# therealadityashankar/hey-buddy

Hardware: AMD Instinct MI355X
Metric: audio clips/sec featurized+trained, 1.5 s @16 kHz, 1/2/4/8 GPU (higher is better)
Workload: dtype f32

## Files before the change

hey-buddy_amd/csrc/hbk_augment.hip:

```cpp
#include <algorithm>
#include <cmath>
#include <numeric>
#include <type_traits>
#include <vector>

#include "hbk_common.h"

namespace hbk {
namespace {

constexpr int kT = 23040;
constexpr int kM = kT / 2;
constexpr int kThreads = 1024;
constexpr int kN1 = 16000;
constexpr int kM1 = kN1 / 2;

template <bool INV>
__device__ __forceinline__ cf tw_const(double frac) {
  const double a = (INV ? 2.0 : -2.0) * M_PI * frac;
  return cf{static_cast<float>(cos(a)), static_cast<float>(sin(a))};
}

template <bool INV>
__device__ __forceinline__ void dft3(cf& a, cf& b, cf& c) {
// ... 1314 lines not shown
#endif

struct PitchArgs {
  const float* x;
  int64_t x_stride;
  const int32_t* idx;
  int n;
  float* out;
  int64_t out_stride;
  int L, f_in, f_out, l1, orig, nw, width, target;
  double rate;
  float* y;
  float* taps;
  int2* yr;
  int span;
};

__device__ __forceinline__ int ps_i0(const PitchArgs& a, int t, float& alpha) {
  const float ts = static_cast<float>(static_cast<double>(t) * a.rate);
  const float fl = floorf(ts);
  alpha = ts - fl;
  return static_cast<int>(fl);
}

struct PvClip {
  float d[kPvRows][8];
  float xs[256];
  float gh[2][kPvGh][8];
  int cnt0;
  int lo, hi;
// ... 105 lines not shown
        }
      }
    }
    done = 4 * n4;
  }
  for (int p = done + lane; p < L; p += 128) {
    if (xr[p] != 0.f) {
      lo = min(lo, p);
      hi = max(hi, p);
    }
  }
  if (hi >= 0) {
    atomicMin(&C.lo, lo);
    atomicMax(&C.hi, hi);
  }
}

#ifdef HBK_PHASE_TIMING
#define HBK_PVT(i)                                     \
  do {                                                 \
    const unsigned long long t_ = __builtin_amdgcn_s_memtime(); \
    pvt[i] += t_ - pvt_t0;                             \
    pvt_t0 = t_;                                       \
  } while (0)
#else
#define HBK_PVT(i) \
  do {             \
  } while (0)
#endif

#ifndef HBK_PV_UNROLL_TAIL
#define HBK_PV_UNROLL_TAIL 1
#endif
#ifndef HBK_PV_WAVES
#define HBK_PV_WAVES 4
#endif
__global__ void __launch_bounds__(128 * kPvClips) __attribute__((amdgpu_waves_per_eu(HBK_PV_WAVES)))
ps_vocoder_kernel(PitchArgs a) {
#ifdef HBK_PHASE_TIMING
  unsigned long long pvt[5] = {0, 0, 0, 0, 0}, pvt_t0 = __builtin_amdgcn_s_memtime();
#endif
  extern __shared__ __attribute__((aligned(16))) unsigned char pv_smem[];
  PvShared& sh = *reinterpret_cast<PvShared*>(pv_smem);
  const int tid = threadIdx.x, cl = tid >> 7, lane = tid & 127;
  const int e = min(static_cast<int>(blockIdx.x) * kPvClips + cl, a.n - 1);
  const bool live = static_cast<int>(blockIdx.x) * kPvClips + cl < a.n;
  const float* xr = a.x + static_cast<int64_t>(a.idx[e]) * a.x_stride;
  PvClip& C = sh.c[cl];
  for (int q = tid; q < 256; q += blockDim.x) {
    double sn, cs;
    sincospi(2.0 * q / kPsFft, &sn, &cs);
    sh.tw[q] = cf{static_cast<float>(cs), static_cast<float>(sn)};
    sh.tw64[q][0] = cs;
    sh.tw64[q][1] = -sn;
  }
  if (lane == 0) C.cnt0 = 0;
  if (lane == 0) {
    C.lo = INT_MAX;
    C.hi = -1;
  }
  __syncthreads();
  if (a.span) pv_scan_span(C, xr, a.L, lane);
  int nz = 0;
  for (int q = lane; q < kPsFft; q += 128) {
    const float v = ps_xp(xr, a.L, q);
    C.xs[q] = v;
    nz += v != 0.f;
  }
  if (nz) atomicAdd(&C.cnt0, nz);
  for (int q = tid; q < 3 * 128; q += blockDim.x) {
    const int j = 2 * (q / 128) + 1, kk = min(q % 128, kPsBins - 1), q1 = (kk * j) % kPsFft,
              q2 = (kk * (j + 1)) % kPsFft;
    sh.wt[q / 128][q % 128] = float4{static_cast<float>(sh.tw64[q1][0]), static_cast<float>(sh.tw64[q1][1]),
                                     static_cast<float>(sh.tw64[q2][0]), static_cast<float>(sh.tw64[q2][1])};
  }
  int fb = 1;
  pv_load_rows(a, sh, xr, cl, lane, fb);
// ... 81 lines not shown
    commit(nre, nim, ncnt);
    cntn = cnt;
    polar(na, nm);
    slide_to(nre, nim, ncnt, C.d[sf + 1 - fb]);
    commit(nre, nim, ncnt);
    polar(pa, pm);
  }
  int c = 0;
  cf R = {1.f, 0.f};
  cf Q = {0.f, 0.f};
  int qz = 0;
  const int dq = q7;
  const cf e7 = sh.tw[q7];
  const int jmax = (a.l1 + kPsPad - 1) / kPsHop;
  float* y = a.y + static_cast<int64_t>(e) * a.l1;
  auto frames_of = [&](int lo, int hi, int& tb, int& tl) {
    tb = 0;
    tl = jmax;
    float al;
    if (lo > hi) {
      tl = -1;
      return;
    }
    if (lo > 2 * kPsPad && a.rate < 2.0) {
      const int fz = (lo - kPsPad) / kPsHop - 1;
      int tg = min(static_cast<int>((fz - 2) / a.rate), a.f_out - 1) & ~(kPvGroup - 1);
      while (tg > 0 && ps_i0(a, tg - 1, al) + 2 > fz) tg -= kPvGroup;
      tb = max(tg, 0);
    }
    if (hi < a.L - 1 - 2 * kPsPad) {
      const int fn = min((hi + kPsPad) / kPsHop, a.f_in - 1);
      int t = max(min(a.f_out - 1, static_cast<int>((fn + 1) / a.rate) + 1), 0);
      while (t > 0 && ps_i0(a, t, al) > fn) --t;
      while (t + 1 < a.f_out && ps_i0(a, t + 1, al) <= fn) ++t;
      tl = min(jmax, t + 36);
    }
  };
  int t_beg = 0, t_last = jmax;
  {
    int tb = 0, tl = jmax;
    if (a.span) {
      int lo = INT_MAX, hi = -1;
      for (int i = 0; i < kPvClips; ++i) {
        lo = min(lo, sh.c[i].lo);
        hi = max(hi, sh.c[i].hi);
      }
      frames_of(lo, hi, t_beg, t_last);
      frames_of(C.lo, C.hi, tb, tl);
    }
    if (lane == 0 && live)
      a.yr[e] = tl < tb ? int2{0, 0}
                        : int2{max(kPsHop * tb - kPsPad, 0), min(kPsHop * (tl + 1) - kPsPad, a.l1)};
// ... 811 lines not shown
      a.rate * kPvGroup + 3 > kPvRows) {
    set_error("hbk: pitch shift %d/%d resamples %d -> %d (%d taps): the kernel holds <= %d phases of <= %d taps "
              "(torch_pitch_shift's fast shifts at 16 kHz)", num, den, a.orig, a.nw, 2 * a.width + a.orig,
              kPsPhaseMax, kPsTapMax);
    return HBK_ERR_UNSUPPORTED;
  }
  return HBK_OK;
}

static int64_t ps_bytes(const hbk::PitchArgs& a, int64_t n, int64_t* off) {
  using namespace hbk;
  auto up = [](int64_t b) { return (b + 255) & ~int64_t(255); };
  off[0] = off[1] = off[2] = off[3] = 0;
  off[4] = up(n * a.l1 * 4);
  off[5] = off[4] + up(int64_t(kPsPhaseMax) * kPsTapMax * 4);
  return off[5] + up(n * int64_t(sizeof(int2)));
}

int64_t hbk_pitch_shift_workspace_size(int64_t n, int64_t T, int32_t sample_rate, int32_t num, int32_t den) {
  hbk::PitchArgs a{};
  if (n <= 0 || ps_geometry(T, sample_rate, num, den, a) != HBK_OK) return 0;
  int64_t off[6];
  return ps_bytes(a, n, off);
}

int hbk_pitch_shift(const float* x, int64_t x_stride, int64_t n, const int32_t* idx, int64_t T, int32_t sample_rate,
                    int32_t num, int32_t den, float* out, int64_t out_stride, void* workspace,
                    int64_t workspace_bytes, void* stream) {
  using namespace hbk;
  if (n < 0) return arg_error("negative n");
  if (n == 0) return HBK_OK;
  if (n > 65535) return arg_error("n > 65535 per call");
  if (!x || !idx || !out || !workspace) return arg_error("NULL pointer");
  PitchArgs a{};
  const int rc = ps_geometry(T, sample_rate, num, den, a);
  if (rc != HBK_OK) return rc;
  if (x_stride < T || out_stride < T) return arg_error("stride < T");
  int64_t off[6];
  if (workspace_bytes < ps_bytes(a, n, off)) return arg_error("workspace too small (hbk_pitch_shift_workspace_size)");
  unsigned char* w = static_cast<unsigned char*>(workspace);
  a.x = x;
  a.x_stride = x_stride;
  a.idx = idx;
  a.out = out;
  a.out_stride = out_stride;
  a.n = static_cast<int>(n);
  a.y = reinterpret_cast<float*>(w + off[3]);
  a.taps = reinterpret_cast<float*>(w + off[4]);
  a.yr = reinterpret_cast<int2*>(w + off[5]);
  static const bool span_off = [] {
    const char* s = getenv("HBK_PS_SPAN");
    return s && s[0] == '0';
  }();
  a.span = span_off ? 0 : 1;
  hipStream_t st = as_stream(stream);
  hipLaunchKernelGGL(ps_taps_kernel, dim3(unsigned((a.nw * kPsTapMax + 255) / 256)), dim3(256), 0, st, a);
  HBK_LAUNCH_CHECK("ps_taps_kernel");
  static bool lds_set = false;
  if (!lds_set) {
    HBK_HIP(hipFuncSetAttribute(reinterpret_cast<const void*>(ps_vocoder_kernel),
                                hipFuncAttributeMaxDynamicSharedMemorySize, int(sizeof(PvShared))));
    lds_set = true;
  }
  hipLaunchKernelGGL(ps_vocoder_kernel, dim3(unsigned((n + kPvClips - 1) / kPvClips)), dim3(128 * kPvClips),
                     sizeof(PvShared), st, a);
  HBK_LAUNCH_CHECK("ps_vocoder_kernel");
  const int res_frames = (a.L + a.nw - 1) / a.nw;
  static const bool valu_rs = getenv("HBK_PS_RESAMPLE_VALU") != nullptr;
  if (valu_rs || a.nw > 128) {
    hipLaunchKernelGGL(ps_resample_kernel, dim3(unsigned((res_frames + kPsResFrames - 1) / kPsResFrames), unsigned(n)),
                       dim3(128), 0, st, a);
    HBK_LAUNCH_CHECK("ps_resample_kernel");
// ... 20 lines not shown
```

hey-buddy_amd/csrc/hbk_mlp.hip:

```cpp
#include <algorithm>
#include <cmath>
#include <vector>

#include "hbk_common.h"
#include "hbk_mlp_internal.h"

namespace hbk {
namespace {

typedef float f4 __attribute__((ext_vector_type(4)));

constexpr int kStats = 8;
constexpr float kLnEps = 1e-5f;

constexpr int GBM = 64, GBN = 64, GBK = 16;

template <bool TA, bool TB>
__global__ void __launch_bounds__(256) gemm_kernel(const float* __restrict__ A, const float* __restrict__ B,
                                                   float* __restrict__ C, const float* __restrict__ bias,
                                                   int M, int N, int K, int lda, int ldb, int ldc,
                                                   int accumulate, int k_split) {
  __shared__ float As[GBK][GBM + 4];
  __shared__ float Bs[GBK][GBN + 4];
  const int tid = threadIdx.x, lane = tid & 63, wave = tid >> 6;
// ... 664 lines not shown
  if (!mlp_fused_supported(*p)) {
    set_error("hbk: the evaluation pass covers the fused plans");
    return HBK_ERR_UNSUPPORTED;
  }
  if (rows < 0 || row_offset < 0 || rows + row_offset > (int64_t(1) << 31) / 768) return arg_error("rows out of range");
  if (rows == 0) return HBK_OK;
  if (!pool || n_pool <= 0) return arg_error("empty pool");
  if (label != 0 && label != 1) return arg_error("label must be 0 or 1");
  if (dropout_p < 0.f || dropout_p >= 1.f) return arg_error("dropout_p must be in [0, 1)");
  if (ws_bytes < mlp_eval_ws_floats(*p, rows) * int64_t(sizeof(float))) return arg_error("workspace too small");
  return mlp_eval_count(*p, params, pool, pool_is_f16 != 0, n_pool, idx, rows, row_offset, label,
                        activation_threshold, dropout_p, seed, counts, prob, static_cast<float*>(workspace),
                        as_stream(stream));
}

int hbk_mlp_eval_count_multi(const hbk_mlp_plan* p, const float* params, int32_t n_pools,
                             const void* const* pools, int32_t pools_are_f16, const int64_t* n_pool,
                             const int64_t* rows, const int64_t* row_offsets, const int32_t* labels,
                             const uint64_t* seeds, float* const* counts, float activation_threshold,
                             float dropout_p, void* workspace, int64_t ws_bytes, void* stream) {
  using namespace hbk;
  if (!p || !params || !workspace) return arg_error("NULL pointer");
  if (!mlp_fused_supported(*p)) {
    set_error("hbk: the evaluation pass covers the fused plans");
    return HBK_ERR_UNSUPPORTED;
  }
  if (n_pools < 0 || n_pools > kEvalMaxSeg) return arg_error("n_pools must be in [0, 4]");
  if (n_pools == 0) return HBK_OK;
  if (!pools || !n_pool || !rows || !row_offsets || !labels || !seeds || !counts) return arg_error("NULL array");
  if (dropout_p < 0.f || dropout_p >= 1.f) return arg_error("dropout_p must be in [0, 1)");
// ... 28 lines not shown
```

hey-buddy_amd/csrc/hbk_mlp_fused.hip:

```cpp
#include <hip/hip_runtime.h>

#include <algorithm>
#include <initializer_list>
#include <utility>
#include <cmath>
#include <cstdio>

#include "hbk_common.h"
#include "hbk_mlp_internal.h"

namespace hbk {
namespace {

typedef float f4 __attribute__((ext_vector_type(4)));
typedef _Float16 h4 __attribute__((ext_vector_type(4)));

constexpr int kD = 1536, kL = 96, kH = 64, kH2 = 128;
constexpr int kR = 16;
constexpr int kMaxG = 4;
constexpr int kStats = 8;
constexpr float kLnEps = 1e-5f;
constexpr int kLd = 132;
constexpr int kChunkMax = 384;

// ... 2101 lines not shown
  const float* P;
  int64_t b_hg[kMaxG], b_o[kMaxG], w_o[kMaxG], ln_g[kMaxG], ln_b[kMaxG];
  const _Float16* wc;
  int64_t c_o[kMaxG], c_hg[kMaxG];
  float act_thr;
  float* counts;
  int label;
  float* prob;
  int nseg;
  int seg_tile0[kKvMaxSeg + 1];
  const void* seg_pool[kKvMaxSeg];
  int64_t seg_npool[kKvMaxSeg], seg_rows[kKvMaxSeg], seg_r0[kKvMaxSeg];
  uint64_t seg_seed[kKvMaxSeg];
  float* seg_counts[kKvMaxSeg];
  int seg_label[kKvMaxSeg];
};

__global__ void __launch_bounds__(256) kv_prep_kernel(const float* __restrict__ P, int64_t w0, int64_t g_in,
                                                      int64_t b_in, _Float16* __restrict__ wq, float* c0,
                                                      float* c1) {
  __shared__ double red[2][4];
  const int n = blockIdx.x, tid = threadIdx.x;
  const float* W = P + w0 + int64_t(n) * kD;
  double s0 = 0.0, s1 = 0.0;
  for (int k = 2 * tid; k < kD; k += 512) {
    const float wa = W[k], wb = W[k + 1];
    const float ga = wa * P[g_in + k], gb = wb * P[g_in + k + 1];
    uint32_t hi, lo;
    split_pair(16.f * ga, 16.f * gb, hi, lo);
    *reinterpret_cast<uint32_t*>(wq + int64_t(n) * kD + k) = hi;
// ... 24 lines not shown
#define HBK_KV_NT 1
#endif
typedef uint32_t u32x4 __attribute__((ext_vector_type(4)));
__device__ __forceinline__ uint4 load_rows4(const uint4* p) {
#if HBK_KV_NT
  const u32x4 v = __builtin_nontemporal_load(reinterpret_cast<const u32x4*>(p));
  return uint4{v[0], v[1], v[2], v[3]};
#else
  return *p;
#endif
}

constexpr int kKvPiece = 8;
__device__ __forceinline__ int kv_swz(int n) { return (n >> 1) & 7; }
constexpr int kNetWLd = 104, kAld = 100;
template <bool kF16, int NG, int W>
__global__ void __launch_bounds__(64 * W) kv_gemm_kernel(KvArgs a0) {
  KvArgs a = a0;
  int blk = static_cast<int>(blockIdx.x);
  if (a0.nseg > 0) {
    int sg = 0;
#pragma unroll
    for (int q = 1; q < kKvMaxSeg; ++q) sg += (q < a0.nseg && blk >= a0.seg_tile0[q]) ? 1 : 0;
    blk -= a0.seg_tile0[sg];
    a.pool = a0.seg_pool[sg];
    a.n_pool = a0.seg_npool[sg];
    a.idx = nullptr;
    a.rows = a0.seg_rows[sg];
    a.r0 = a0.seg_r0[sg];
    a.seed = a0.seg_seed[sg];
    a.counts = a0.seg_counts[sg];
    a.label = a0.seg_label[sg];
    a.prob = nullptr;
  }
  constexpr int kWBuf = 3;
  constexpr int kRT = (kF16 && W == 8) ? 2 : 1;
  constexpr int kThr = 64 * W;
  constexpr int kGemmBytes = kWBuf * 2 * kH2 * kKvKC * 2;
  constexpr int kWsBytes = 2 * kH2 * kNetWLd * 2;
  constexpr int kActBytes = W * 16 * kRT * kAld * 4;
  constexpr int kLdsBytes = (kGemmBytes > kWsBytes + kActBytes ? kGemmBytes : kWsBytes + kActBytes) + 16;
  static_assert(kLdsBytes <= 160 * 1024, "one workgroup's LDS");
  __shared__ __attribute__((aligned(16))) unsigned char smem[kLdsBytes];
  auto wb = reinterpret_cast<_Float16 (*)[2][kH2][kKvKC]>(smem);
  float (*stS)[16 * kRT][2] = reinterpret_cast<float (*)[16 * kRT][2]>(smem);
  static_assert(sizeof(float) * W * 16 * kRT * 2 <= kWsBytes, "statistics: below the activation tiles");
#ifndef HBK_KV_DEPTH
#define HBK_KV_DEPTH 2
#endif
  constexpr int kDepth = kF16 ? HBK_KV_DEPTH : 2;
  constexpr int kBGroup = kDepth > 2 ? 2 : 4;
  constexpr int kU = kF16 ? 1 : 2;
  constexpr int kALoads = kRT * 2 * kU;
  constexpr int kTile = W * 16 * kRT;
  constexpr int kDma = 32 / W;
  static_assert(kALoads * (kDepth - 1) + kDma < 16, "the counted waits use vmcnt's low field");
  const int tid = threadIdx.x, lane = tid & 63, wave = tid >> 6, m = lane & 15, kq = lane >> 4;
  const int64_t tile0 = int64_t(blk) * kTile;
  const char* rp[kRT];
  uint32_t rid[kRT];
#pragma unroll
  for (int rt = 0; rt < kRT; ++rt) {
    const int64_t r = min(tile0 + 16 * kRT * wave + 16 * rt + m, a.rows - 1);
    int64_t pr = a.idx ? static_cast<int64_t>(a.idx[r]) : (a.r0 + r) % a.n_pool;
    pr = min(max(pr, int64_t(0)), a.n_pool - 1);
    rp[rt] = static_cast<const char*>(a.pool) + pr * kD * (kF16 ? 2 : 4);
    rid[rt] = static_cast<uint32_t>(a.r0 + r);
  }
  const uint64_t seed = a.seed;
  const uint32_t s0 = static_cast<uint32_t>(seed), s1 = static_cast<uint32_t>(seed >> 32) * 0x27D4EB2Fu;
  const uint32_t thr = static_cast<uint32_t>(a.drop_p * 65536.f + 0.5f);
  const float keep = a.drop_p > 0.f ? 1.f / (1.f - a.drop_p) : 1.f;
  uint4 ar[kDepth][kRT][2][kU];
  auto load_rows = [&](int c, int slot) {
#pragma unroll
    for (int rt = 0; rt < kRT; ++rt)
#pragma unroll
      for (int kb = 0; kb < 2; ++kb) {
        const int k = kKvKC * c + 32 * kb + 8 * kq;
#pragma unroll
        for (int u = 0; u < kU; ++u)
          ar[slot][rt][kb][u] = load_rows4(reinterpret_cast<const uint4*>(rp[rt] + int64_t(k) * (kF16 ? 2 : 4) + 16 * u));
      }
  };
  auto dma_w = [&](int c, int buf) {
#pragma unroll
    for (int j = 0; j < kDma; ++j) {
      const int row8 = kDma * wave + j;
      const int pl = row8 >> 4, n = 8 * (row8 & 15) + (lane >> 3), pc = (lane & 7) ^ kv_swz(n);
      const _Float16* src = a.wq + int64_t(pl) * kH2 * kD + int64_t(n) * kD + kKvKC * c + kKvPiece * pc;
      __builtin_amdgcn_global_load_lds(src, &wb[buf][pl][8 * (row8 & 15)][0], 16, 0, 0);
// ... 20 lines not shown
  for (int cb = 0; cb < kKvChunks; cb += kDepth)
#pragma unroll
  for (int slot = 0; slot < kDepth; ++slot) {
    const int c = cb + slot;
    const int bnext = buf == 0 ? kWBuf - 1 : buf - 1;
    h8 ah[kRT][2], al[kRT][2];
    float t1[kRT], t2[kRT];
#pragma unroll
    for (int rt = 0; rt < kRT; ++rt) t1[rt] = t2[rt] = 0.f;
#pragma unroll
    for (int kb = 0; kb < 2; ++kb)
#pragma unroll
      for (int rt = 0; rt < kRT; ++rt) {
        float v[8];
        if (kF16) {
          const h8 hv = __builtin_bit_cast(h8, ar[slot][rt][kb][0]);
#pragma unroll
          for (int e = 0; e < 8; ++e) v[e] = static_cast<float>(hv[e]);
        } else {
#pragma unroll
          for (int e = 0; e < 8; ++e) v[e] = __builtin_bit_cast(float, (&ar[slot][rt][kb][e >> 2].x)[e & 3]);
        }
        if (!(HBK_KV_ABLATE & 2) && a.drop_p > 0.f) {
          const uint32_t base = rid[rt] * (kD / 2) + ((kKvKC * c + 32 * kb + 8 * kq) >> 1);
#pragma unroll
          for (int e = 0; e < 8; e += 2) {
            const uint32_t hsh = drop_hash(s0, s1, base + (e >> 1));
            v[e] = (hsh & 0xFFFFu) < thr ? 0.f : v[e];
            v[e + 1] = (hsh >> 16) < thr ? 0.f : v[e + 1];
          }
        }
#pragma unroll
        for (int e = 0; e < 8; ++e) {
          t1[rt] += v[e];
          t2[rt] += v[e] * v[e];
        }
// ... 225 lines not shown
  {
    const int r = lane >> 2, c0 = 16 * (lane & 3);
    float wo[16];
#pragma unroll
    for (int q = 0; q < 16; ++q) wo[q] = P[a.w_o[NG - 1] + c0 + q];
    const float bz = P[a.b_o[NG - 1]];
    int ge = 0, gt = 0;
#pragma unroll
    for (int rt = 0; rt < kRT; ++rt) {
      float z = 0.f;
#pragma unroll
      for (int q = 0; q < 16; ++q) z = fmaf(A[(16 * rt + r) * kAld + c0 + q], wo[q], z);
      z += dpp_f<0xB1>(z);
      z += dpp_f<0x4E>(z);
      z += bz;
      const int64_t row = tile0 + 16 * kRT * wave + 16 * rt + r;
      const bool live = row < a.rows && (lane & 3) == 0;
      const float p = sigm_fast(z);
      if (live && a.prob) a.prob[row] = p;
      ge += __popcll(__ballot(live && p >= a.act_thr));
      gt += __popcll(__ballot(live && p > a.act_thr));
    }
    if (lane == 0) {
      if (ge) atomicAdd(&cntS[0], static_cast<float>(ge));
      if (gt) atomicAdd(&cntS[1], static_cast<float>(gt));
    }
  }
  lds_barrier();
  if (tid < 2 && cntS[tid] != 0.f) atomicAdd(a.counts + 2 * a.label + tid, cntS[tid]);
}


// ... 632 lines not shown

int mlp_eval_prepare(const hbk_mlp_plan& p, const float* params, float* ws, hipStream_t s) {
  const int NG = static_cast<int>(p.g.size());
  const EvalWs w = eval_layout(NG);
  const WSplit wsp = make_wsplit(p);
  const int64_t n4 = wsplit_halves(NG) / 16;
  hipLaunchKernelGGL(k0_wsplit_kernel, dim3(unsigned(std::min<int64_t>((n4 + 255) / 256, 256))), dim3(256), 0, s,
                     wsp, params, reinterpret_cast<_Float16*>(ws + w.wsplit), n4);
  HBK_LAUNCH_CHECK("k0_wsplit_kernel");
  hipLaunchKernelGGL(kv_prep_kernel, dim3(kH2), dim3(256), 0, s, params, p.g[0].w_hg, p.ln_in.g, p.ln_in.b,
                     reinterpret_cast<_Float16*>(ws + w.wq), ws + w.c0, ws + w.c1);
  HBK_LAUNCH_CHECK("kv_prep_kernel");
  return HBK_OK;
}

static int mlp_eval_launch(const hbk_mlp_plan& p, const float* params, bool f16, const EvalSeg* seg, int nseg,
                           const int32_t* idx, float act_thr, float drop_p, float* prob, float* ws, hipStream_t s) {
  const int NG = static_cast<int>(p.g.size());
  const EvalWs w = eval_layout(NG);
  const WSplit wsp = make_wsplit(p);
  K2Args kc{};
  set_k2_cache(wsp, NG, reinterpret_cast<const _Float16*>(ws + w.wsplit), kc);
  KvArgs ka{};
  ka.pool = seg[0].pool;
  ka.n_pool = seg[0].n_pool;
  ka.idx = idx;
  ka.rows = seg[0].rows;
  ka.r0 = seg[0].r0;
  ka.wq = reinterpret_cast<const _Float16*>(ws + w.wq);
  ka.c0 = ws + w.c0;
// ... 25 lines not shown
    ka.nseg = nseg;
    tiles = 0;
    for (int i = 0; i < nseg; ++i) {
      ka.seg_tile0[i] = static_cast<int>(tiles);
      ka.seg_pool[i] = seg[i].pool;
      ka.seg_npool[i] = seg[i].n_pool;
      ka.seg_rows[i] = seg[i].rows;
      ka.seg_r0[i] = seg[i].r0;
      ka.seg_seed[i] = seg[i].seed;
      ka.seg_counts[i] = seg[i].counts;
      ka.seg_label[i] = seg[i].label;
      tiles += (seg[i].rows + tile - 1) / tile;
    }
    ka.seg_tile0[nseg] = static_cast<int>(tiles);
  }
  const dim3 grid(static_cast<unsigned>(tiles));
  auto launch = [&](auto kern) { hipLaunchKernelGGL(kern, grid, dim3(64 * waves), 0, s, ka); };
  if (waves == 16) {
    if (NG == 2) launch(kv_gemm_kernel<true, 2, 16>);
    else if (NG == 3) launch(kv_gemm_kernel<true, 3, 16>);
    else launch(kv_gemm_kernel<true, 4, 16>);
  } else if (f16) {
    if (NG == 2) launch(kv_gemm_kernel<true, 2, 8>);
    else if (NG == 3) launch(kv_gemm_kernel<true, 3, 8>);
    else launch(kv_gemm_kernel<true, 4, 8>);
  } else {
    if (NG == 2) launch(kv_gemm_kernel<false, 2, 8>);
    else if (NG == 3) launch(kv_gemm_kernel<false, 3, 8>);
    else launch(kv_gemm_kernel<false, 4, 8>);
  }
// ... 70 lines not shown
```

hey-buddy_amd/csrc/hbk_mlp_internal.h:

```cpp
#pragma once

#include <hip/hip_runtime.h>
#include <stdint.h>

#include <vector>

namespace hbk {

struct Gmlp {
  int in, hid, out;
  int64_t w_hg, b_hg, w_o, b_o;
};
struct Ln {
  int d;
  int64_t g, b;
};

}

struct hbk_mlp_plan {
  int d_in = 0, layer = 0, hid = 0, n_layers = 0;
  hbk::Ln ln_in;
  std::vector<hbk::Gmlp> g;
  std::vector<hbk::Ln> ln;
// ... 20 lines not shown
int64_t mlp_fused_ws_floats(const hbk_mlp_plan& p, int64_t B);
int mlp_fused_step_variant(int64_t B, hipStream_t s);
int mlp_fused_run(const hbk_mlp_plan& p, const float* params, const float* pool32, int64_t n32,
                  const void* pool16, int64_t n16, const int32_t* idx, int64_t idx_stride, int64_t idx_steps,
                  const float* y, int64_t y_stride, int B, const float* state, int parity, const float* sched,
                  int sched_len, float neg_weight, float thr, float act_thr, float drop_p, uint64_t seed,
                  float* bucket, float* prob, float* logit, float* ws, bool train, int flags, hipStream_t s);
int mlp_fused_update(const hbk_mlp_plan& p, float* params, float* bucket, float* m, float* v, float* state,
                     int parity, const float* sched, int sched_len, float lr, float b1, float b2, float eps,
                     float* hist, int hist_cap, float* ws, hipStream_t s);
int64_t mlp_eval_ws_floats(const hbk_mlp_plan& p, int64_t rows);
int mlp_eval_prepare(const hbk_mlp_plan& p, const float* params, float* ws, hipStream_t s);
int mlp_eval_count(const hbk_mlp_plan& p, const float* params, const void* pool, bool f16, int64_t n_pool,
                   const int32_t* idx, int64_t rows, int64_t r0, int label, float act_thr, float drop_p,
                   uint64_t seed, float* counts, float* prob, float* ws, hipStream_t s);
struct EvalSeg {
  const void* pool;
  int64_t n_pool, rows, r0;
  uint64_t seed;
  float* counts;
  int label;
};
constexpr int kEvalMaxSeg = 4;
int mlp_eval_count_multi(const hbk_mlp_plan& p, const float* params, bool f16, const EvalSeg* seg, int nseg,
                         float act_thr, float drop_p, float* ws, hipStream_t s);
int mlp_eval_finish(const float* cv, const float* ct, const double* sizes, float target, float ratio, float* sched,
                    int64_t sched_len, int64_t next_step, float* out, hipStream_t s);
}
```

hey-buddy_amd/heybuddy/_native.py:

```python
from __future__ import annotations

import ctypes
import os
import threading
from typing import Optional

import torch

__all__ = ["HBKError", "HBKUnavailable", "lib", "check", "stream_ptr", "require_device",
           "LIB_PATH"]

LIB_PATH = os.environ.get(
    "HBK_LIB",
    os.path.join(os.path.dirname(os.path.dirname(os.path.abspath(__file__))), "lib", "libhbk.so"),
)


class HBKError(RuntimeError):
    """A libhbk.so entry point returned a non-zero status."""


class HBKUnavailable(HBKError):
    """libhbk.so (or a HIP device) is not available: the HIP path cannot run."""

# ... 74 lines not shown
    "hbk_mlp_fused_supported": (_c_int, [_vp, ctypes.POINTER(ctypes.c_int32)]),
    "hbk_mlp_step_variant": (_c_int, [_vp, _c_int64, _vp, ctypes.POINTER(ctypes.c_int32)]),
    "hbk_mlp_step_fwd_bwd": (_c_int, [_vp, _vp, _vp, _c_int64, _vp, _c_int64, _vp, _c_int64, _vp, _c_int64,
                                      _c_int64, _vp, ctypes.c_int32, _vp, _c_int64, _c_float, _c_float,
                                      _c_float, _c_float, ctypes.c_uint64, _vp, _vp, _c_int64, ctypes.c_int32,
                                      _vp, _c_int64, _vp]),
    "hbk_mlp_step_update": (_c_int, [_vp, _vp, _vp, _vp, _vp, _vp, ctypes.c_int32, _vp, _c_int64, _c_float,
                                     _c_float, _c_float, _c_float, _vp, ctypes.c_int32, _vp, _c_int64, _vp]),
    "hbk_mlp_eval_workspace_size": (_c_int, [_vp, _c_int64, ctypes.POINTER(_c_int64)]),
    "hbk_mlp_eval_prepare": (_c_int, [_vp, _vp, _vp, _c_int64, _vp]),
    "hbk_mlp_eval_count_multi": (_c_int, [_vp, _vp, ctypes.c_int32, _vp, ctypes.c_int32, _vp, _vp, _vp, _vp, _vp,
                                          _vp, _c_float, _c_float, _vp, _c_int64, _vp]),
    "hbk_mlp_eval_count": (_c_int, [_vp, _vp, _vp, ctypes.c_int32, _c_int64, _vp, _c_int64, _c_int64,
                                    ctypes.c_int32, _c_float, _c_float, ctypes.c_uint64, _vp, _vp, _vp, _c_int64,
                                    _vp]),
    "hbk_mlp_eval_finish": (_c_int, [_vp, _vp, ctypes.POINTER(ctypes.c_double), _c_float, _c_float, _vp,
                                     _c_int64, _c_int64, _vp, _vp]),
}


class GraphOp(ctypes.Structure):
    _fields_ = [
        ("kind", ctypes.c_int32), ("kh", ctypes.c_int32), ("kw", ctypes.c_int32),
        ("cin", ctypes.c_int32), ("cout", ctypes.c_int32), ("act", ctypes.c_int32),
        ("alpha", ctypes.c_float), ("weight", _vp), ("bias", _vp),
    ]


def exported_symbols() -> list[str]:
    return list(_PROTOS)
# ... 52 lines not shown
```

hey-buddy_amd/heybuddy/kernels.py:

```python
from __future__ import annotations

import ctypes
import os
import itertools
import threading
from typing import Dict

import numpy as np
import torch

from heybuddy import _native
from heybuddy._native import check, lib, ptr, stream_ptr

__all__ = ["MelPlan", "mel_frames"]

_plans: Dict[int, object] = {}
_plan_ids = itertools.count(1)
_plans_lock = threading.Lock()


def _register(plan) -> int:
    with _plans_lock:
        pid = next(_plan_ids)
        _plans[pid] = plan
# ... 458 lines not shown
        flat = pool.reshape(pool.shape[0], -1)
        if flat.shape[1] != self.d_in or pool.dtype not in (torch.float32, torch.float16) or pool.device != dev \
                or not pool.is_contiguous():
            raise ValueError(f"pool must be a contiguous [n, {self.d_in}] f32 / f16 tensor on {dev}")
        if idx is not None and (idx.dtype != torch.int32 or idx.device != dev or not idx.is_contiguous()
                                or idx.numel() < rows):
            raise ValueError("idx must be a contiguous int32 device tensor of >= rows entries")
        if counts.dtype != torch.float32 or counts.numel() < 4 or counts.device != dev:
            raise ValueError("counts must be a float32 [4] device tensor")
        if prob is not None and (prob.dtype != torch.float32 or prob.numel() < rows or prob.device != dev):
            raise ValueError("prob must be a float32 device tensor of >= rows entries")
        torch.ops.hbk.mlp_eval_count_(params, pool, idx, int(rows), int(row_offset), int(label),
                                      float(activation_threshold), float(dropout_p), _u64_to_i64(seed), counts, prob,
                                      ws, self.id)

    def eval_count_multi(self, params: torch.Tensor, parts, counts: torch.Tensor, ws: torch.Tensor,
                         activation_threshold: float = 0.5, dropout_p: float = 0.0) -> None:
        dev = params.device
        if not 0 < len(parts) <= 4:
            raise ValueError("1 to 4 pools per launch")
        dt = parts[0][0].dtype
        for pool, rows, _, label, which, _ in parts:
            if pool.dtype != dt or pool.dtype not in (torch.float32, torch.float16) or pool.device != dev \
                    or not pool.is_contiguous() or pool.reshape(pool.shape[0], -1).shape[1] != self.d_in:
                raise ValueError(f"pools must be contiguous [n, {self.d_in}] tensors of one dtype on {dev}")
            if label not in (0, 1) or which not in (0, 1) or rows < 0:
                raise ValueError("label / which must be 0 or 1, rows >= 0")
        if counts.dtype != torch.float32 or counts.shape != (2, 4) or counts.device != dev \
                or not counts.is_contiguous():
            raise ValueError("counts must be a contiguous float32 [2, 4] device tensor")
# ... 570 lines not shown
```

include/hbk.h:

```cpp
#ifndef HBK_H
#define HBK_H

#include <stdint.h>

#ifdef __cplusplus
extern "C" {
#endif

typedef enum {
  HBK_OK = 0,
  HBK_ERR_ARG = -1,
  HBK_ERR_HIP = -2,
  HBK_ERR_UNSUPPORTED = -3
} hbk_status;

const char* hbk_version(void);
const char* hbk_last_error(void);
int hbk_device_count(int* count);
int hbk_stream_create_cu_mask(const uint32_t* cu_mask, int n_words, void** stream);
int hbk_stream_destroy(void* stream);

int hbk_profile_mark(int32_t tag, void* stream);

typedef struct hbk_mel_plan hbk_mel_plan;
// ... 95 lines not shown
                         void* workspace, int64_t workspace_bytes, void* stream);
int hbk_mlp_step_update(const hbk_mlp_plan* plan, float* params, float* bucket, float* m, float* v,
                        float* state, int32_t parity, const float* sched, int64_t sched_len, float lr,
                        float beta1, float beta2, float eps, float* history, int32_t history_cap,
                        void* workspace, int64_t workspace_bytes, void* stream);

int hbk_mlp_set_step_scalars(hbk_mlp_plan* plan, const double* dev_scalars);

int hbk_mlp_eval_workspace_size(const hbk_mlp_plan* plan, int64_t rows, int64_t* bytes);
int hbk_mlp_eval_prepare(const hbk_mlp_plan* plan, const float* params, void* workspace, int64_t workspace_bytes,
                         void* stream);
int hbk_mlp_eval_count(const hbk_mlp_plan* plan, const float* params, const void* pool, int32_t pool_is_f16,
                       int64_t n_pool, const int32_t* idx, int64_t rows, int64_t row_offset, int32_t label,
                       float activation_threshold, float dropout_p, uint64_t seed, float* counts, float* prob,
                       void* workspace, int64_t workspace_bytes, void* stream);
int hbk_mlp_eval_count_multi(const hbk_mlp_plan* plan, const float* params, int32_t n_pools,
                             const void* const* pools, int32_t pools_are_f16, const int64_t* n_pool,
                             const int64_t* rows, const int64_t* row_offsets, const int32_t* labels,
                             const uint64_t* seeds, float* const* counts, float activation_threshold,
                             float dropout_p, void* workspace, int64_t workspace_bytes, void* stream);
int hbk_mlp_eval_finish(const float* counts_val, const float* counts_test, const double* sizes,
                        float target_false_positives_per_hour, float adjust_ratio, float* sched, int64_t sched_len,
                        int64_t next_step, float* out, void* stream);

typedef struct hbk_reverb_plan hbk_reverb_plan;

int hbk_reverb_plan_create(int64_t T, hbk_reverb_plan** plan);
int hbk_reverb_plan_destroy(hbk_reverb_plan* plan);

#define HBK_REVERB_SPECTRUM_SLOTS 11536
// ... 57 lines not shown
```

Before: 1.046 million.

## Sort pitch-shift clips by nonzero span and add lap-form MLP eval kernel

Result: faster. 1.070 million (median of 6 runs) (+2.3%).

```diff
diff --git a/hey-buddy_amd/csrc/hbk_augment.hip b/hey-buddy_amd/csrc/hbk_augment.hip
--- a/hey-buddy_amd/csrc/hbk_augment.hip
+++ b/hey-buddy_amd/csrc/hbk_augment.hip
@@ -1352,6 +1352,10 @@
   float* taps;
   int2* yr;
   int span;
+  int2* sp;
+  uint64_t* key;
+  int32_t* ord;
+  int32_t* gord;
 };
 
 __device__ __forceinline__ int ps_i0(const PitchArgs& a, int t, float& alpha) {
@@ -1487,6 +1491,124 @@
     atomicMin(&C.lo, lo);
     atomicMax(&C.hi, hi);
   }
+}
+
+__device__ __forceinline__ void pv_frames_of(const PitchArgs& a, int lo, int hi, int& tb, int& tl) {
+  const int jmax = (a.l1 + kPsPad - 1) / kPsHop;
+  tb = 0;
+  tl = jmax;
+  float al;
+  if (lo > hi) {
+    tl = -1;
+    return;
+  }
+  if (lo > 2 * kPsPad && a.rate < 2.0) {
+    const int fz = (lo - kPsPad) / kPsHop - 1;
+    int tg = min(static_cast<int>((fz - 2) / a.rate), a.f_out - 1) & ~(kPvGroup - 1);
+    while (tg > 0 && ps_i0(a, tg - 1, al) + 2 > fz) tg -= kPvGroup;
+    tb = max(tg, 0);
+  }
+  if (hi < a.L - 1 - 2 * kPsPad) {
+    const int fn = min((hi + kPsPad) / kPsHop, a.f_in - 1);
+    int t = max(min(a.f_out - 1, static_cast<int>((fn + 1) / a.rate) + 1), 0);
+    while (t > 0 && ps_i0(a, t, al) > fn) --t;
+    while (t + 1 < a.f_out && ps_i0(a, t + 1, al) <= fn) ++t;
+    tl = min(jmax, t + 36);
+  }
+}
+
+constexpr int kPsQuant = 360;
+
+__global__ void __launch_bounds__(256) ps_span_kernel(PitchArgs a) {
+  const int lane = threadIdx.x & 63, e = blockIdx.x * 4 + (threadIdx.x >> 6);
+  if (e >= a.n) return;
+  const float* xr = a.x + static_cast<int64_t>(a.idx[e]) * a.x_stride;
+  constexpr int kChunk = 64 * 8;
+  int lo = INT_MAX, hi = -1;
+  for (int p0 = 0; p0 < a.L; p0 += kChunk) {
+    float v[8];
+#pragma unroll
+    for (int j = 0; j < 8; ++j) {
+      const int p = p0 + 64 * j + lane;
+      v[j] = p < a.L ? xr[p] : 0.f;
+    }
+#pragma unroll
+    for (int j = 0; j < 8; ++j)
+      if (v[j] != 0.f) {
+        lo = min(lo, p0 + 64 * j + lane);
+        hi = max(hi, p0 + 64 * j + lane);
+      }
+    if (__any(hi >= 0)) break;
+  }
+  for (int o = 32; o >= 1; o >>= 1) {
+    lo = min(lo, __shfl_xor(lo, o, 64));
+    hi = max(hi, __shfl_xor(hi, o, 64));
+  }
+  if (hi >= 0) {
+    for (int p1 = a.L; p1 > hi + 1; p1 -= kChunk) {
+      float v[8];
+      int h = -1;
+#pragma unroll
+      for (int j = 0; j < 8; ++j) {
+        const int p = p1 - kChunk + 64 * j + lane;
+        v[j] = (p > hi && p < a.L) ? xr[max(p, 0)] : 0.f;
+      }
+#pragma unroll
+      for (int j = 0; j < 8; ++j)
+        if (v[j] != 0.f) h = max(h, p1 - kChunk + 64 * j + lane);
+      if (__any(h >= 0)) {
+        for (int o = 32; o >= 1; o >>= 1) h = max(h, __shfl_xor(h, o, 64));
+        hi = h;
+        break;
+      }
+    }
+  }
+  if (lane == 0) {
+    a.sp[e] = int2{lo, hi};
+    const uint64_t q = hi < 0 ? 0 : 1 + static_cast<uint64_t>(hi / kPsQuant), f = hi < 0 ? 0 : static_cast<uint64_t>(lo);
+    a.key[e] = (q << 40) | (f << 16) | static_cast<uint64_t>(e);
+  }
+}
+
+__global__ void __launch_bounds__(1024) ps_rank_kernel(const uint64_t* __restrict__ key, int n,
+                                                       int32_t* __restrict__ ord) {
+  __shared__ int part[16][64];
+  const int lane = threadIdx.x & 63, w = threadIdx.x >> 6, i = blockIdx.x * 64 + lane;
+  const uint64_t mine = key[min(i, n - 1)];
+  const int per = (n + 15) / 16, j0 = min(w * per, n), j1 = min(j0 + per, n);
+  int below = 0;
+  for (int jb = j0; jb < j1; jb += 64) {
+    const uint64_t kl = jb + lane < j1 ? key[jb + lane] : ~uint64_t(0);
+#pragma unroll
+    for (int q = 0; q < 64; ++q) {
+      const uint32_t hi = __builtin_amdgcn_readlane(static_cast<int>(kl >> 32), q);
+      const uint32_t lo = __builtin_amdgcn_readlane(static_cast<int>(kl), q);
+      below += ((static_cast<uint64_t>(hi) << 32) | lo) < mine;
+    }
+  }
+  part[w][lane] = below;
+  __syncthreads();
+  if (w == 0 && i < n) {
+    int r = 0;
+#pragma unroll
+    for (int q = 0; q < 16; ++q) r += part[q][lane];
+    ord[r] = i;
+  }
+}
+
+__global__ void __launch_bounds__(256) ps_group_kernel(PitchArgs a, int groups) {
+  const int g = blockIdx.x * 256 + threadIdx.x;
+  if (g >= groups) return;
+  int lo = INT_MAX, hi = -1;
+  for (int c = 0; c < kPvClips; ++c) {
+    const int2 s = a.sp[a.ord[min(kPvClips * g + c, a.n - 1)]];
+    lo = min(lo, s.x);
+    hi = max(hi, s.y);
+  }
+  int tb, tl;
+  pv_frames_of(a, lo, hi, tb, tl);
+  const int steps = tl < tb ? 0 : (tl - tb) / kPvGroup + 1;
+  a.key[g] = (static_cast<uint64_t>((1 << 24) - steps) << 16) | static_cast<uint64_t>(g);
 }
 
 #ifdef HBK_PHASE_TIMING
@@ -1516,8 +1638,9 @@
   extern __shared__ __attribute__((aligned(16))) unsigned char pv_smem[];
   PvShared& sh = *reinterpret_cast<PvShared*>(pv_smem);
   const int tid = threadIdx.x, cl = tid >> 7, lane = tid & 127;
-  const int e = min(static_cast<int>(blockIdx.x) * kPvClips + cl, a.n - 1);
-  const bool live = static_cast<int>(blockIdx.x) * kPvClips + cl < a.n;
+  const int slot = (a.sp ? a.gord[blockIdx.x] : static_cast<int>(blockIdx.x)) * kPvClips + cl;
+  const int e = a.sp ? a.ord[min(slot, a.n - 1)] : min(slot, a.n - 1);
+  const bool live = slot < a.n;
   const float* xr = a.x + static_cast<int64_t>(a.idx[e]) * a.x_stride;
   PvClip& C = sh.c[cl];
   for (int q = tid; q < 256; q += blockDim.x) {
@@ -1529,11 +1652,12 @@
   }
   if (lane == 0) C.cnt0 = 0;
   if (lane == 0) {
-    C.lo = INT_MAX;
-    C.hi = -1;
+    const int2 s = a.sp ? a.sp[e] : int2{INT_MAX, -1};
+    C.lo = s.x;
+    C.hi = s.y;
   }
   __syncthreads();
-  if (a.span) pv_scan_span(C, xr, a.L, lane);
+  if (a.span && !a.sp) pv_scan_span(C, xr, a.L, lane);
   int nz = 0;
   for (int q = lane; q < kPsFft; q += 128) {
     const float v = ps_xp(xr, a.L, q);
@@ -1645,28 +1769,7 @@
   const cf e7 = sh.tw[q7];
   const int jmax = (a.l1 + kPsPad - 1) / kPsHop;
   float* y = a.y + static_cast<int64_t>(e) * a.l1;
-  auto frames_of = [&](int lo, int hi, int& tb, int& tl) {
-    tb = 0;
-    tl = jmax;
-    float al;
-    if (lo > hi) {
-      tl = -1;
-      return;
-    }
-    if (lo > 2 * kPsPad && a.rate < 2.0) {
-      const int fz = (lo - kPsPad) / kPsHop - 1;
-      int tg = min(static_cast<int>((fz - 2) / a.rate), a.f_out - 1) & ~(kPvGroup - 1);
-      while (tg > 0 && ps_i0(a, tg - 1, al) + 2 > fz) tg -= kPvGroup;
-      tb = max(tg, 0);
-    }
-    if (hi < a.L - 1 - 2 * kPsPad) {
-      const int fn = min((hi + kPsPad) / kPsHop, a.f_in - 1);
-      int t = max(min(a.f_out - 1, static_cast<int>((fn + 1) / a.rate) + 1), 0);
-      while (t > 0 && ps_i0(a, t, al) > fn) --t;
-      while (t + 1 < a.f_out && ps_i0(a, t + 1, al) <= fn) ++t;
-      tl = min(jmax, t + 36);
-    }
-  };
+  auto frames_of = [&](int lo, int hi, int& tb, int& tl) { pv_frames_of(a, lo, hi, tb, tl); };
   int t_beg = 0, t_last = jmax;
   {
     int tb = 0, tl = jmax;
@@ -2508,13 +2611,17 @@
   off[0] = off[1] = off[2] = off[3] = 0;
   off[4] = up(n * a.l1 * 4);
   off[5] = off[4] + up(int64_t(kPsPhaseMax) * kPsTapMax * 4);
-  return off[5] + up(n * int64_t(sizeof(int2)));
+  off[6] = off[5] + up(n * int64_t(sizeof(int2)));
+  off[7] = off[6] + up(n * int64_t(sizeof(int2)));
+  off[8] = off[7] + up(n * int64_t(sizeof(uint64_t)));
+  off[9] = off[8] + up(n * int64_t(sizeof(int32_t)));
+  return off[9] + up(n * int64_t(sizeof(int32_t)));
 }
 
 int64_t hbk_pitch_shift_workspace_size(int64_t n, int64_t T, int32_t sample_rate, int32_t num, int32_t den) {
   hbk::PitchArgs a{};
   if (n <= 0 || ps_geometry(T, sample_rate, num, den, a) != HBK_OK) return 0;
-  int64_t off[6];
+  int64_t off[10];
   return ps_bytes(a, n, off);
 }
 
@@ -2530,7 +2637,7 @@
   const int rc = ps_geometry(T, sample_rate, num, den, a);
   if (rc != HBK_OK) return rc;
   if (x_stride < T || out_stride < T) return arg_error("stride < T");
-  int64_t off[6];
+  int64_t off[10];
   if (workspace_bytes < ps_bytes(a, n, off)) return arg_error("workspace too small (hbk_pitch_shift_workspace_size)");
   unsigned char* w = static_cast<unsigned char*>(workspace);
   a.x = x;
@@ -2547,9 +2654,26 @@
     return s && s[0] == '0';
   }();
   a.span = span_off ? 0 : 1;
+  const char* pair_env = getenv("HBK_PS_PAIR");
+  const bool pair = a.span && !(pair_env && pair_env[0] == '0');
   hipStream_t st = as_stream(stream);
   hipLaunchKernelGGL(ps_taps_kernel, dim3(unsigned((a.nw * kPsTapMax + 255) / 256)), dim3(256), 0, st, a);
   HBK_LAUNCH_CHECK("ps_taps_kernel");
+  const int groups = static_cast<int>((n + kPvClips - 1) / kPvClips);
+  if (pair) {
+    a.sp = reinterpret_cast<int2*>(w + off[6]);
+    a.key = reinterpret_cast<uint64_t*>(w + off[7]);
+    a.ord = reinterpret_cast<int32_t*>(w + off[8]);
+    a.gord = reinterpret_cast<int32_t*>(w + off[9]);
+    hipLaunchKernelGGL(ps_span_kernel, dim3(unsigned((n + 3) / 4)), dim3(256), 0, st, a);
+    HBK_LAUNCH_CHECK("ps_span_kernel");
+    hipLaunchKernelGGL(ps_rank_kernel, dim3(unsigned((n + 63) / 64)), dim3(1024), 0, st, static_cast<const uint64_t*>(a.key), a.n, a.ord);
+    HBK_LAUNCH_CHECK("ps_rank_kernel");
+    hipLaunchKernelGGL(ps_group_kernel, dim3(unsigned((groups + 255) / 256)), dim3(256), 0, st, a, groups);
+    HBK_LAUNCH_CHECK("ps_group_kernel");
+    hipLaunchKernelGGL(ps_rank_kernel, dim3(unsigned((groups + 63) / 64)), dim3(1024), 0, st, static_cast<const uint64_t*>(a.key), groups, a.gord);
+    HBK_LAUNCH_CHECK("ps_rank_kernel");
+  }
   static bool lds_set = false;
   if (!lds_set) {
     HBK_HIP(hipFuncSetAttribute(reinterpret_cast<const void*>(ps_vocoder_kernel),
diff --git a/hey-buddy_amd/csrc/hbk_mlp.hip b/hey-buddy_amd/csrc/hbk_mlp.hip
--- a/hey-buddy_amd/csrc/hbk_mlp.hip
+++ b/hey-buddy_amd/csrc/hbk_mlp.hip
@@ -702,6 +702,14 @@
                         as_stream(stream));
 }
 
+int hbk_mlp_eval_laps(int64_t rows, int64_t n_pool, int32_t pool_is_f16, int32_t has_idx, int64_t* parts) {
+  using namespace hbk;
+  if (!parts) return arg_error("NULL pointer");
+  if (rows < 0 || n_pool <= 0) return arg_error("rows / n_pool out of range");
+  mlp_eval_lap_plan(rows, n_pool, pool_is_f16 != 0, has_idx != 0, parts);
+  return HBK_OK;
+}
+
 int hbk_mlp_eval_count_multi(const hbk_mlp_plan* p, const float* params, int32_t n_pools,
                              const void* const* pools, int32_t pools_are_f16, const int64_t* n_pool,
                              const int64_t* rows, const int64_t* row_offsets, const int32_t* labels,
diff --git a/hey-buddy_amd/csrc/hbk_mlp_fused.hip b/hey-buddy_amd/csrc/hbk_mlp_fused.hip
--- a/hey-buddy_amd/csrc/hbk_mlp_fused.hip
+++ b/hey-buddy_amd/csrc/hbk_mlp_fused.hip
@@ -2139,6 +2139,7 @@
   uint64_t seg_seed[kKvMaxSeg];
   float* seg_counts[kKvMaxSeg];
   int seg_label[kKvMaxSeg];
+  int lap_tiles;
 };
 
 __global__ void __launch_bounds__(256) kv_prep_kernel(const float* __restrict__ P, int64_t w0, int64_t g_in,
@@ -2193,8 +2194,9 @@
 constexpr int kKvPiece = 8;
 __device__ __forceinline__ int kv_swz(int n) { return (n >> 1) & 7; }
 constexpr int kNetWLd = 104, kAld = 100;
-template <bool kF16, int NG, int W>
+template <bool kF16, int NG, int W, int kLap = 0>
 __global__ void __launch_bounds__(64 * W) kv_gemm_kernel(KvArgs a0) {
+  static_assert(kLap == 0 || (kF16 && W == 8 && kLap == 2), "the lap form: f16 rows, 8 waves of two laps");
   KvArgs a = a0;
   int blk = static_cast<int>(blockIdx.x);
   if (a0.nseg > 0) {
@@ -2213,7 +2215,8 @@
     a.prob = nullptr;
   }
   constexpr int kWBuf = 3;
-  constexpr int kRT = (kF16 && W == 8) ? 2 : 1;
+  constexpr int kRT = kLap ? kLap : (kF16 && W == 8) ? 2 : 1;
+  constexpr int kAT = kLap ? 1 : kRT;
   constexpr int kThr = 64 * W;
   constexpr int kGemmBytes = kWBuf * 2 * kH2 * kKvKC * 2;
   constexpr int kWsBytes = 2 * kH2 * kNetWLd * 2;
@@ -2230,14 +2233,34 @@
   constexpr int kDepth = kF16 ? HBK_KV_DEPTH : 2;
   constexpr int kBGroup = kDepth > 2 ? 2 : 4;
   constexpr int kU = kF16 ? 1 : 2;
-  constexpr int kALoads = kRT * 2 * kU;
+  constexpr int kALoads = kAT * 2 * kU;
   constexpr int kTile = W * 16 * kRT;
   constexpr int kDma = 32 / W;
   static_assert(kALoads * (kDepth - 1) + kDma < 16, "the counted waits use vmcnt's low field");
   const int tid = threadIdx.x, lane = tid & 63, wave = tid >> 6, m = lane & 15, kq = lane >> 4;
   const int64_t tile0 = int64_t(blk) * kTile;
-  const char* rp[kRT];
+  const int64_t lap_s = kLap ? int64_t(blk / max(a.lap_tiles, 1)) * kLap * a.n_pool : 0;
+  const int64_t lap_b = kLap ? int64_t(blk % max(a.lap_tiles, 1)) * (16 * W) + 16 * wave : 0;
+  auto row_of = [&](int rt, int j, bool& live) -> int64_t {
+    if constexpr (kLap > 0) {
+      const int64_t r = lap_s + rt * a.n_pool + lap_b + j;
+      live = lap_b + j < a.n_pool && r < a.rows;
+      return r;
+    } else {
+      const int64_t r = tile0 + 16 * kRT * wave + 16 * rt + j;
+      live = r < a.rows;
+      return r;
+    }
+  };
+  const char* rp[kAT];
   uint32_t rid[kRT];
+  if constexpr (kLap > 0) {
+    const int64_t b = min(lap_b + m, a.n_pool - 1);
+    const int64_t pr = min(max((a.r0 + b) % a.n_pool, int64_t(0)), a.n_pool - 1);
+    rp[0] = static_cast<const char*>(a.pool) + pr * kD * 2;
+#pragma unroll
+    for (int rt = 0; rt < kRT; ++rt) rid[rt] = static_cast<uint32_t>(a.r0 + lap_s + rt * a.n_pool + b);
+  } else {
 #pragma unroll
   for (int rt = 0; rt < kRT; ++rt) {
     const int64_t r = min(tile0 + 16 * kRT * wave + 16 * rt + m, a.rows - 1);
@@ -2246,14 +2269,15 @@
     rp[rt] = static_cast<const char*>(a.pool) + pr * kD * (kF16 ? 2 : 4);
     rid[rt] = static_cast<uint32_t>(a.r0 + r);
   }
+  }
   const uint64_t seed = a.seed;
   const uint32_t s0 = static_cast<uint32_t>(seed), s1 = static_cast<uint32_t>(seed >> 32) * 0x27D4EB2Fu;
   const uint32_t thr = static_cast<uint32_t>(a.drop_p * 65536.f + 0.5f);
   const float keep = a.drop_p > 0.f ? 1.f / (1.f - a.drop_p) : 1.f;
-  uint4 ar[kDepth][kRT][2][kU];
+  uint4 ar[kDepth][kAT][2][kU];
   auto load_rows = [&](int c, int slot) {
 #pragma unroll
-    for (int rt = 0; rt < kRT; ++rt)
+    for (int rt = 0; rt < kAT; ++rt)
 #pragma unroll
       for (int kb = 0; kb < 2; ++kb) {
         const int k = kKvKC * c + 32 * kb + 8 * kq;
@@ -2304,12 +2328,12 @@
       for (int rt = 0; rt < kRT; ++rt) {
         float v[8];
         if (kF16) {
-          const h8 hv = __builtin_bit_cast(h8, ar[slot][rt][kb][0]);
+          const h8 hv = __builtin_bit_cast(h8, ar[slot][kLap ? 0 : rt][kb][0]);
 #pragma unroll
           for (int e = 0; e < 8; ++e) v[e] = static_cast<float>(hv[e]);
         } else {
 #pragma unroll
-          for (int e = 0; e < 8; ++e) v[e] = __builtin_bit_cast(float, (&ar[slot][rt][kb][e >> 2].x)[e & 3]);
+          for (int e = 0; e < 8; ++e) v[e] = __builtin_bit_cast(float, (&ar[slot][kLap ? 0 : rt][kb][e >> 2].x)[e & 3]);
         }
         if (!(HBK_KV_ABLATE & 2) && a.drop_p > 0.f) {
           const uint32_t base = rid[rt] * (kD / 2) + ((kKvKC * c + 32 * kb + 8 * kq) >> 1);
@@ -2565,8 +2589,9 @@
       z += dpp_f<0xB1>(z);
       z += dpp_f<0x4E>(z);
       z += bz;
-      const int64_t row = tile0 + 16 * kRT * wave + 16 * rt + r;
-      const bool live = row < a.rows && (lane & 3) == 0;
+      bool live;
+      const int64_t row = row_of(rt, r, live);
+      live = live && (lane & 3) == 0;
       const float p = sigm_fast(z);
       if (live && a.prob) a.prob[row] = p;
       ge += __popcll(__ballot(live && p >= a.act_thr));
@@ -3229,6 +3254,15 @@
   return HBK_OK;
 }
 
+void mlp_eval_lap_plan(int64_t rows, int64_t n_pool, bool f16, bool has_idx, int64_t part[2]) {
+  part[0] = 0;
+  part[1] = rows;
+  const char* e = getenv("HBK_EVAL_LAPS");
+  if ((e && e[0] == '0') || !f16 || has_idx || n_pool <= 0 || rows <= 0) return;
+  part[0] = rows / (2 * n_pool) * (2 * n_pool);
+  part[1] = rows - part[0];
+}
+
 static int mlp_eval_launch(const hbk_mlp_plan& p, const float* params, bool f16, const EvalSeg* seg, int nseg,
                            const int32_t* idx, float act_thr, float drop_p, float* prob, float* ws, hipStream_t s) {
   const int NG = static_cast<int>(p.g.size());
@@ -3284,6 +3318,26 @@
     }
     ka.seg_tile0[nseg] = static_cast<int>(tiles);
   }
+  if (nseg == 1) {
+    int64_t part[2];
+    mlp_eval_lap_plan(seg[0].rows, seg[0].n_pool, f16, idx != nullptr, part);
+    if (part[0] > 0) {
+      ka.lap_tiles = static_cast<int>((seg[0].n_pool + 127) / 128);
+      ka.rows = part[0];
+      const dim3 lgrid(static_cast<unsigned>(part[0] / (2 * seg[0].n_pool) * ka.lap_tiles));
+      auto llaunch = [&](auto kern) { hipLaunchKernelGGL(kern, lgrid, dim3(512), 0, s, ka); };
+      if (NG == 2) llaunch(kv_gemm_kernel<true, 2, 8, 2>);
+      else if (NG == 3) llaunch(kv_gemm_kernel<true, 3, 8, 2>);
+      else llaunch(kv_gemm_kernel<true, 4, 8, 2>);
+      HBK_LAUNCH_CHECK("kv_gemm_kernel (laps)");
+      ka.r0 += part[0];
+      if (ka.prob) ka.prob += part[0];
+      ka.lap_tiles = 0;
+      ka.rows = part[1];
+      if (part[1] == 0) return HBK_OK;
+      tiles = (part[1] + tile - 1) / tile;
+    }
+  }
   const dim3 grid(static_cast<unsigned>(tiles));
   auto launch = [&](auto kern) { hipLaunchKernelGGL(kern, grid, dim3(64 * waves), 0, s, ka); };
   if (waves == 16) {
diff --git a/hey-buddy_amd/csrc/hbk_mlp_internal.h b/hey-buddy_amd/csrc/hbk_mlp_internal.h
--- a/hey-buddy_amd/csrc/hbk_mlp_internal.h
+++ b/hey-buddy_amd/csrc/hbk_mlp_internal.h
@@ -58,6 +58,7 @@
 int mlp_eval_count(const hbk_mlp_plan& p, const float* params, const void* pool, bool f16, int64_t n_pool,
                    const int32_t* idx, int64_t rows, int64_t r0, int label, float act_thr, float drop_p,
                    uint64_t seed, float* counts, float* prob, float* ws, hipStream_t s);
+void mlp_eval_lap_plan(int64_t rows, int64_t n_pool, bool f16, bool has_idx, int64_t part[2]);
 struct EvalSeg {
   const void* pool;
   int64_t n_pool, rows, r0;
diff --git a/hey-buddy_amd/heybuddy/_native.py b/hey-buddy_amd/heybuddy/_native.py
--- a/hey-buddy_amd/heybuddy/_native.py
+++ b/hey-buddy_amd/heybuddy/_native.py
@@ -112,6 +112,8 @@
     "hbk_mlp_eval_count": (_c_int, [_vp, _vp, _vp, ctypes.c_int32, _c_int64, _vp, _c_int64, _c_int64,
                                     ctypes.c_int32, _c_float, _c_float, ctypes.c_uint64, _vp, _vp, _vp, _c_int64,
                                     _vp]),
+    "hbk_mlp_eval_laps": (_c_int, [_c_int64, _c_int64, ctypes.c_int32, ctypes.c_int32,
+                                   ctypes.POINTER(_c_int64)]),
     "hbk_mlp_eval_finish": (_c_int, [_vp, _vp, ctypes.POINTER(ctypes.c_double), _c_float, _c_float, _vp,
                                      _c_int64, _c_int64, _vp, _vp]),
 }
diff --git a/hey-buddy_amd/heybuddy/kernels.py b/hey-buddy_amd/heybuddy/kernels.py
--- a/hey-buddy_amd/heybuddy/kernels.py
+++ b/hey-buddy_amd/heybuddy/kernels.py
@@ -496,6 +496,13 @@
                                       float(activation_threshold), float(dropout_p), _u64_to_i64(seed), counts, prob,
                                       ws, self.id)
 
+    @staticmethod
+    def eval_laps(rows: int, n_pool: int, f16: bool = True, has_idx: bool = False) -> tuple:
+        parts = (ctypes.c_int64 * 2)()
+        check(lib().hbk_mlp_eval_laps(int(rows), int(n_pool), int(bool(f16)), int(bool(has_idx)), parts),
+              "hbk_mlp_eval_laps")
+        return tuple(int(v) for v in parts)
+
     def eval_count_multi(self, params: torch.Tensor, parts, counts: torch.Tensor, ws: torch.Tensor,
                          activation_threshold: float = 0.5, dropout_p: float = 0.0) -> None:
         dev = params.device
diff --git a/include/hbk.h b/include/hbk.h
--- a/include/hbk.h
+++ b/include/hbk.h
@@ -133,6 +133,7 @@
                        int64_t n_pool, const int32_t* idx, int64_t rows, int64_t row_offset, int32_t label,
                        float activation_threshold, float dropout_p, uint64_t seed, float* counts, float* prob,
                        void* workspace, int64_t workspace_bytes, void* stream);
+int hbk_mlp_eval_laps(int64_t rows, int64_t n_pool, int32_t pool_is_f16, int32_t has_idx, int64_t* parts);
 int hbk_mlp_eval_count_multi(const hbk_mlp_plan* plan, const float* params, int32_t n_pools,
                              const void* const* pools, int32_t pools_are_f16, const int64_t* n_pool,
                              const int64_t* rows, const int64_t* row_offsets, const int32_t* labels,
```
